# gcallipo/RadioDSP_SDR_RX

Hardware: AMD Instinct MI355X
Metric: IQ Msamples/s through full SSB+NR chain; achieved HBM GB/s vs peak (higher is better)
Workload: dtype f32

## Files before the change

radiodsp_sdr_rx_amd/csrc/rdsp_tail.hip:

```cpp
#include "rdsp_wave.h"

using namespace rdsp;

namespace {

typedef float v2f __attribute__((ext_vector_type(2)));

template <int CTRL>
__device__ __forceinline__ float dpp0_f(float v) {
  return __builtin_bit_cast(
      float, __builtin_amdgcn_update_dpp(0, __builtin_bit_cast(int, v), CTRL, 0xF, 0xF, true));
}

__device__ __forceinline__ float reduce_halves(float a0, float a1) {
  float t;
  asm("s_nop 1\n\t"
      "v_add_f32_dpp %0, %1, %1 row_ror:8 row_mask:0xf bank_mask:0x3\n\t"
      "v_add_f32_dpp %0, %2, %2 row_ror:8 row_mask:0xf bank_mask:0xc\n\t"
      "s_nop 1\n\t"
      "v_add_f32_dpp %0, %0, %0 row_half_mirror row_mask:0xf bank_mask:0xf\n\t"
      "s_nop 1\n\t"
      "v_add_f32_dpp %0, %0, %0 quad_perm:[2,3,0,1] row_mask:0xf bank_mask:0xf\n\t"
      "s_nop 1\n\t"
      "v_add_f32_dpp %0, %0, %0 quad_perm:[1,0,3,2] row_mask:0xf bank_mask:0xf"
      : "=&v"(t)
      : "v"(a0), "v"(a1));
  return t;
}

struct NlmsB {
  static constexpr int TPL = 6, GS = 64, SCR = 3 * GS;
  static constexpr int LDS_SCR = 2 * SCR;
  static constexpr bool OUT_IN_SCR = false;
  v2f w2[TPL / 2];
  v2f P[8];
  float energy;
  float emin;

  static __device__ __forceinline__ v2f pair_ld(const float *mine, int m) { return v2f{mine[m], mine[m + 1]}; }
  static __device__ __forceinline__ v2f pair_ld_even(const float *mine, int m) {
    typedef const volatile __attribute__((address_space(3))) v2f *LP;
    return *(LP)(mine + m);
  }
  __device__ __forceinline__ void load(const float *wst, const float *est, size_t ch, int sub) {
#pragma unroll
    for (int t = 0; t < TPL; t++) w2[t >> 1][t & 1] = wst[ch * RDSP_LMS_TAPS + (95 - (TPL * sub + t))];
    energy = est[ch];
    emin = __builtin_inff();
  }
  __device__ __forceinline__ void store(float *wst, float *est, size_t ch, int sub) {
#pragma unroll
    for (int t = 0; t < TPL; t++) wst[ch * RDSP_LMS_TAPS + (95 - (TPL * sub + t))] = w2[t >> 1][t & 1];
    if (sub == 0) est[ch] = energy;
  }

  static __device__ __forceinline__ void prepare(const float *cur, int s0, int sub, float mu, float e_base,
                                                 float b_base, float *dst, float &emin) {
    const float *x = cur + s0 + 4 * sub;
    const float xm = x[-1], qm = x[-97];
    const float4 xv = *reinterpret_cast<const float4 *>(x), qv = *reinterpret_cast<const float4 *>(x - 96);
    const float xs[5] = {xm, xv.x, xv.y, xv.z, xv.w}, qs[5] = {qm, qv.x, qv.y, qv.z, qv.w};
    float ea[4], ba[4];
#pragma unroll
    for (int k = 0; k < 4; k++) {
      const float de = fmaf(xs[k + 1], xs[k + 1], -(qs[k + 1] * qs[k + 1]));
      const float db = fmaf(xs[k + 1], xs[k], -(qs[k + 1] * qs[k]));
      ea[k] = (k == 0) ? de : ea[k - 1] + de;
      ba[k] = (k == 0) ? db : ba[k - 1] + db;
    }
    float ie = ea[3], ib = ba[3];
    ie += dpp0_f<0x111>(ie); ib += dpp0_f<0x111>(ib);
    ie += dpp0_f<0x112>(ie); ib += dpp0_f<0x112>(ib);
    ie += dpp0_f<0x114>(ie); ib += dpp0_f<0x114>(ib);
    ie += dpp0_f<0x118>(ie); ib += dpp0_f<0x118>(ib);
    const float oe = e_base + (ie - ea[3]), ob = b_base + (ib - ba[3]);
    float e[4], g[4], b[4];
#pragma unroll
    for (int k = 0; k < 4; k++) {
      e[k] = oe + ea[k];
      b[k] = ob + ba[k];
      const float den = e[k] + 0.000000119209289f;
      g[k] = mu * __builtin_amdgcn_rcpf(den);
      emin = fminf(emin, den);
    }
    float4 *d4 = reinterpret_cast<float4 *>(dst);
    d4[sub] = make_float4(g[0], g[1], g[2], g[3]);
    d4[GS / 4 + sub] = make_float4(b[0], b[1], b[2], b[3]);
    d4[GS / 2 + sub] = make_float4(e[0], e[1], e[2], e[3]);
  }

  template <bool OUT_E>
  __device__ __forceinline__ void block(const float *ring, bool first, float mu, float *out, float *scr, int sub, bool running) {
    const float *cur = ring + RDSP_BLOCK;
    const float *dsrc = first ? cur : ring;
    const float *mine = cur - TPL * sub;
    float bb = 0.f, ee = 0.f;
#pragma unroll
    for (int t = 0; t < TPL; t++) {
      bb = fmaf(mine[-1 - t], mine[-2 - t], bb);
      ee = fmaf(mine[-1 - t], mine[-1 - t], ee);
    }
    float b_base = row_allsum(bb);
    float e_base = row_allsum(ee);
    e_base = running ? energy : e_base;
    prepare(cur, 0, sub, mu, e_base, b_base, scr, emin);
#pragma unroll
    for (int m = -5; m <= 0; m++) P[m & 7] = (m & 1) ? pair_ld(mine, m) : pair_ld_even(mine, m);
#pragma unroll 1
    for (int s0 = 0; s0 < RDSP_BLOCK; s0 += GS) {
      const float *sc = scr + ((s0 / GS) & 1) * SCR;
      wg_sync<1>();
      float4 gq = *reinterpret_cast<const float4 *>(sc);
      float4 bq = *reinterpret_cast<const float4 *>(sc + GS);
      float4 dq = *reinterpret_cast<const float4 *>(dsrc + s0);
      e_base = sc[2 * GS + GS - 1];
      b_base = sc[GS + GS - 1];
      if (s0 + GS < RDSP_BLOCK) prepare(cur, s0 + GS, sub, mu, e_base, b_base, scr + (((s0 / GS) + 1) & 1) * SCR, emin);
#pragma unroll
      for (int q = 0; q < GS / 4; q++) {
        const float gi[4] = {gq.x, gq.y, gq.z, gq.w}, bn[4] = {bq.x, bq.y, bq.z, bq.w};
        const float dd[4] = {dq.x, dq.y, dq.z, dq.w};
        if (q < GS / 4 - 1) {
          gq = *reinterpret_cast<const float4 *>(sc + 4 * (q + 1));
          bq = *reinterpret_cast<const float4 *>(sc + GS + 4 * (q + 1));
          dq = *reinterpret_cast<const float4 *>(dsrc + s0 + 4 * (q + 1));
        }
        float o4[4];
#pragma unroll
        for (int h = 0; h < 2; h++) {
          const int n = 4 * q + 2 * h;
          if ((n + 3 < GS) || (s0 + GS < RDSP_BLOCK)) {
            P[(n + 1) & 7] = pair_ld(mine, s0 + n + 1);
            P[(n + 2) & 7] = pair_ld_even(mine, s0 + n + 2);
          }
          v2f acc = v2f{w2[0][0], w2[0][0]} * P[n & 7];
          acc = __builtin_elementwise_fma(v2f{w2[0][1], w2[0][1]}, P[(n - 1) & 7], acc);
          acc = __builtin_elementwise_fma(v2f{w2[1][0], w2[1][0]}, P[(n - 2) & 7], acc);
          acc = __builtin_elementwise_fma(v2f{w2[1][1], w2[1][1]}, P[(n - 3) & 7], acc);
          acc = __builtin_elementwise_fma(v2f{w2[2][0], w2[2][0]}, P[(n - 4) & 7], acc);
          acc = __builtin_elementwise_fma(v2f{w2[2][1], w2[2][1]}, P[(n - 5) & 7], acc);
          const float t = reduce_halves(acc[0], acc[1]);
          const float dA0 = dd[2 * h] - dpp_f<0x150>(t);
          const float dA1 = dd[2 * h + 1] - dpp_f<0x158>(t);
          const float g0 = dA0 * gi[2 * h];
          const float e1 = fmaf(-g0, bn[2 * h + 1], dA1);
          const float g1 = e1 * gi[2 * h + 1];
          o4[2 * h] = OUT_E ? dA0 : dd[2 * h] - dA0;
          o4[2 * h + 1] = OUT_E ? e1 : dd[2 * h + 1] - e1;
          const v2f gg0 = {g0, g0}, gg1 = {g1, g1};
#pragma unroll
          for (int kk = 0; kk < TPL / 2; kk++) {
            const v2f p0 = P[(n - 2 * kk - 1) & 7], p1 = P[(n - 2 * kk) & 7];
            w2[kk] = __builtin_elementwise_fma(gg0, __builtin_shufflevector(p0, p0, 1, 0), w2[kk]);
            w2[kk] = __builtin_elementwise_fma(gg1, __builtin_shufflevector(p1, p1, 1, 0), w2[kk]);
          }
        }
        *reinterpret_cast<float4 *>(out + s0 + 4 * q) = make_float4(o4[0], o4[1], o4[2], o4[3]);
        __builtin_amdgcn_sched_barrier(0);
      }
    }
    energy = e_base;
  }
  static __device__ __forceinline__ float4 out4(const float *out, const float *, int i) {
    return *reinterpret_cast<const float4 *>(out + i);
  }
};

#ifdef RDSP_EXPERIMENTAL
#include "rdsp_tail_lookahead.h"
#endif

template <typename NL>
__device__ __forceinline__ uint32_t nlms_health(const NL &f) {
  float z = f.energy * 0.f;
#pragma unroll
  for (int k = 0; k < NL::TPL / 2; k++) z = fmaf(f.w2[k][0], 0.f, fmaf(f.w2[k][1], 0.f, z));
  const float bad_e = row_allsum(f.emin <= 0.f ? 1.f : 0.f);
  const float nf = row_allsum(z);
  return (bad_e > 0.f ? 1u : 0u) | (nf == 0.f ? 0u : 2u);
}

#ifdef RDSP_TAIL_PROFILE
#define RDSP_TP(i) do { const long long tp_now = __builtin_readcyclecounter(); tp_acc[i] += tp_now - tp_last; tp_last = tp_now; } while (0)
#else
#define RDSP_TP(i) do { } while (0)
#endif

template <bool DUAL, typename NL>
__device__ __forceinline__ void tail_body(const RdspTailParams &p) {
#ifdef RDSP_TAIL_PROFILE
  long long tp_acc[4] = {0, 0, 0, 0}, tp_last = __builtin_readcyclecounter();
#endif
  constexpr int CPW = 4, SPL = RDSP_BLOCK / 16;
  constexpr int RINGS = DUAL ? 2 : 1;
  constexpr int FIN = NL::OUT_IN_SCR ? 0 : RDSP_BLOCK;
  constexpr int PER_CH0 = 2 * RINGS * RDSP_BLOCK + FIN + NL::LDS_SCR;
  constexpr int PER_CH = PER_CH0 + (96 - PER_CH0 % 64) % 64;
  static_assert(PER_CH % 64 == 32 && PER_CH % 4 == 0, "channel pitch in LDS");
  static_assert(!(DUAL && NL::OUT_IN_SCR), "the two-instance kernel hands a block on through `out`");
  __shared__ __attribute__((aligned(16))) float lds[CPW][PER_CH];
  if (p.prio == 1) __builtin_amdgcn_s_setprio(1);
  else if (p.prio == 2) __builtin_amdgcn_s_setprio(2);
  else if (p.prio == 3) __builtin_amdgcn_s_setprio(3);
  const int lane = threadIdx.x;
  const int cw = lane >> 4, sub = lane & 15;
  size_t ch = (size_t)p.ch_base + (size_t)blockIdx.x * CPW + cw;
  const bool valid = ch < (size_t)p.n_channels;
  if (!valid) ch = p.n_channels - 1;

  float *ringA = &lds[cw][0];
  float *ringB = DUAL ? &lds[cw][2 * RDSP_BLOCK] : ringA;
  float *fin = &lds[cw][2 * RINGS * RDSP_BLOCK];
  float *scr = &lds[cw][2 * RINGS * RDSP_BLOCK + FIN];

  const bool has_inst = DUAL || p.nr_on || p.als_mode;
  const bool one_is_nr = !DUAL && p.nr_on;
  float *o_w = one_is_nr ? p.nr_w : p.als_w;
  float *o_prev = one_is_nr ? p.nr_prev : p.als_prev;
  float *o_energy = one_is_nr ? p.nr_energy : p.als_energy;
  const float o_mu = one_is_nr ? p.nr_mu : p.als_mu;
  const int o_first = one_is_nr ? p.nr_first : p.als_first;
  const int o_mode = one_is_nr ? p.nr_mode : p.als_mode;

  NL nr, als;
  if constexpr (DUAL) {
    nr.load(p.nr_w, p.nr_energy, ch, sub);
    als.load(p.als_w, p.als_energy, ch, sub);
  } else if (has_inst) {
    als.load(o_w, o_energy, ch, sub);
  }
  float agc_g = p.st_scal[ch * 4 + 1];

  if constexpr (DUAL) {
#pragma unroll
    for (int k = 0; k < SPL; k++) {
      ringA[sub * SPL + k] = p.nr_prev[ch * RDSP_BLOCK + sub * SPL + k];
      ringB[sub * SPL + k] = p.als_prev[ch * RDSP_BLOCK + sub * SPL + k];
    }
  } else if (has_inst) {
#pragma unroll
    for (int k = 0; k < SPL; k++) ringA[sub * SPL + k] = o_prev[ch * RDSP_BLOCK + sub * SPL + k];
  }
  const float4 *src4 = reinterpret_cast<const float4 *>(p.mid + ch * p.mid_stride + sub * SPL);
  static_assert(SPL == 8, "two float4 per lane and block");
  float4 nx0 = src4[0], nx1 = src4[1];
  __builtin_amdgcn_s_waitcnt(0x0F70);
  if (p.n_blocks > 0) {
    float4 *dst4 = reinterpret_cast<float4 *>(ringA + RDSP_BLOCK + sub * SPL);
    dst4[0] = nx0;
    dst4[1] = nx1;
    if (p.n_blocks > 1) {
      nx0 = src4[RDSP_BLOCK / 4];
      nx1 = src4[RDSP_BLOCK / 4 + 1];
    }
  }

#pragma unroll 1
  for (int b = 0; b < p.n_blocks; b++) {
    wg_sync<1>();
    RDSP_TP(0);
    if constexpr (DUAL) {
      float *o = ringB + RDSP_BLOCK;
      nr.template block<false>(ringA, p.nr_first && b == 0, p.nr_mu, o, scr, sub, p.energy_running != 0);
      wg_sync<1>();
      if (p.nr_mode == 0) {
#pragma unroll
        for (int k = 0; k < SPL; k++) o[sub * SPL + k] = mul_1p1(o[sub * SPL + k]);
        wg_sync<1>();
      }
      if (p.als_mode == 1) als.template block<true>(ringB, p.als_first && b == 0, p.als_mu, fin, scr, sub, p.energy_running != 0);
      else als.template block<false>(ringB, p.als_first && b == 0, p.als_mu, fin, scr, sub, p.energy_running != 0);
    } else if (has_inst) {
      if (o_mode == 1) als.template block<true>(ringA, o_first && b == 0, o_mu, fin, scr, sub, p.energy_running != 0);
      else als.template block<false>(ringA, o_first && b == 0, o_mu, fin, scr, sub, p.energy_running != 0);
    }
    wg_sync<1>();
    RDSP_TP(1);
    float L[SPL];
#pragma unroll
    for (int k = 0; k < SPL / 4; k++) {
      const float4 a = has_inst ? NL::out4(fin, scr, sub * SPL + 4 * k)
                                : *reinterpret_cast<const float4 *>(ringA + RDSP_BLOCK + sub * SPL + 4 * k);
      L[4 * k] = a.x; L[4 * k + 1] = a.y; L[4 * k + 2] = a.z; L[4 * k + 3] = a.w;
    }
    if (!DUAL && has_inst && o_mode == 0) {
#pragma unroll
      for (int k = 0; k < SPL; k++) L[k] = mul_1p1(L[k]);
    }
    if (b + 1 < p.n_blocks) {
      float4 *r4 = reinterpret_cast<float4 *>(ringA + sub * SPL);
#pragma unroll
      for (int k = 0; k < SPL / 4; k++) r4[k] = r4[RDSP_BLOCK / 4 + k];
      if constexpr (DUAL) {
        float4 *q4 = reinterpret_cast<float4 *>(ringB + sub * SPL);
#pragma unroll
        for (int k = 0; k < SPL / 4; k++) q4[k] = q4[RDSP_BLOCK / 4 + k];
      }
      r4[RDSP_BLOCK / 4] = nx0;
      r4[RDSP_BLOCK / 4 + 1] = nx1;
      if (b + 2 < p.n_blocks) {
        const float4 *n4 = src4 + (size_t)(b + 2) * (RDSP_BLOCK / 4);
        nx0 = n4[0];
        nx1 = n4[1];
      }
    }
    RDSP_TP(2);
    if (p.raw_out) {
      if (valid) {
#pragma unroll
        for (int k = 0; k < SPL; k++)
          p.raw_out[ch * p.mid_stride + (size_t)b * RDSP_BLOCK + sub * SPL + k] = L[k];
      }
      wg_sync<1>();
      continue;
    }
    if (p.agc_on) {
      float pw = 0.f;
#pragma unroll
      for (int k = 0; k < SPL; k++) pw += L[k] * L[k] + L[k] * L[k];
      pw = row_allsum(pw);
      float pp = pw / (float)(2 * RDSP_BLOCK);
      float rms = __builtin_amdgcn_sqrtf(pp);
      float gt = fminf(0.25f * __builtin_amdgcn_rcpf(rms + 1e-6f), 100.0f);
      float coef = (gt < agc_g) ? p.agc_attack : p.agc_decay;
      float gn = agc_g + coef * (gt - agc_g);
#pragma unroll
      for (int k = 0; k < SPL; k++) {
        int i = sub * SPL + k;
        float gg = agc_g + (gn - agc_g) * ((float)(i + 1) / (float)RDSP_BLOCK);
        L[k] *= gg;
      }
      agc_g = gn;
    }
    if (valid) {
      size_t o = ch * p.out_stride + (size_t)b * RDSP_BLOCK + sub * SPL;
#pragma unroll
      for (int k = 0; k < SPL; k += 4) {
        uint4 wv;
        float l0 = L[k] * p.out_gain, l1 = L[k + 1] * p.out_gain, l2 = L[k + 2] * p.out_gain,
              l3 = L[k + 3] * p.out_gain;
        wv.x = pack_lr(l0, l0); wv.y = pack_lr(l1, l1); wv.z = pack_lr(l2, l2); wv.w = pack_lr(l3, l3);
        *reinterpret_cast<uint4 *>(p.out_i16 + o + k) = wv;
        if (p.out_f32) {
          p.out_f32[o + k] = make_float2(l0, l0);
          p.out_f32[o + k + 1] = make_float2(l1, l1);
          p.out_f32[o + k + 2] = make_float2(l2, l2);
          p.out_f32[o + k + 3] = make_float2(l3, l3);
        }
      }
    }
    wg_sync<1>();
    RDSP_TP(3);
  }
#ifdef RDSP_TAIL_PROFILE
  if (p.out_f32 == nullptr && blockIdx.x == 0 && threadIdx.x == 0)
    printf("tail phases (cycles per 128-step block): top %lld  nlms %lld  rotate %lld  agc/pack %lld\n", tp_acc[0] / p.n_blocks,
           tp_acc[1] / p.n_blocks, tp_acc[2] / p.n_blocks, tp_acc[3] / p.n_blocks);
#endif

  if (p.st_status && has_inst) {
    uint32_t h_nr = 0, h_als = 0;
    if constexpr (DUAL) {
      h_nr = nlms_health(nr);
      h_als = nlms_health(als);
    } else if (one_is_nr) {
      h_nr = nlms_health(als);
    } else {
      h_als = nlms_health(als);
    }
    if (valid && sub == 0) {
      if (h_nr) p.st_status[ch] |= h_nr;
      if (h_als) p.st_status[p.st_status_stride + ch] |= h_als;
    }
  }
  if (valid) {
    if constexpr (DUAL) {
      nr.store(p.nr_w, p.nr_energy, ch, sub);
      als.store(p.als_w, p.als_energy, ch, sub);
#pragma unroll
      for (int k = 0; k < SPL; k++) {
        p.nr_prev[ch * RDSP_BLOCK + sub * SPL + k] = ringA[RDSP_BLOCK + sub * SPL + k];
        p.als_prev[ch * RDSP_BLOCK + sub * SPL + k] = ringB[RDSP_BLOCK + sub * SPL + k];
      }
    } else if (has_inst) {
      als.store(o_w, o_energy, ch, sub);
#pragma unroll
      for (int k = 0; k < SPL; k++) o_prev[ch * RDSP_BLOCK + sub * SPL + k] = ringA[RDSP_BLOCK + sub * SPL + k];
    }
    if (sub == 0 && !p.raw_out) p.st_scal[ch * 4 + 1] = agc_g;
  }
}

__global__ void __launch_bounds__(64) rdsp_tail_dual_kernel(RdspTailParams p) { tail_body<true, NlmsB>(p); }

__global__ void __launch_bounds__(64) rdsp_tail_kernel(RdspTailParams p) {
  tail_body<false, NlmsB>(p);
}
#ifdef RDSP_EXPERIMENTAL
__global__ void __launch_bounds__(64) __attribute__((amdgpu_num_vgpr(64))) rdsp_tail_lookahead_kernel(RdspTailParams p) {
  tail_body<false, NlmsL>(p);
}
__global__ void __launch_bounds__(64) __attribute__((amdgpu_num_vgpr(64))) rdsp_tail_four_kernel(RdspTailParams p) {
  tail_body<false, NlmsQ>(p);
}
#endif

}

#ifdef RDSP_EXPERIMENTAL
extern "C" int rdsp_launch_tail_shift(const RdspTailParams *p, hipStream_t stream);
extern "C" int rdsp_launch_tail_layouts(const RdspTailParams *p, int variant, hipStream_t stream);
#endif

extern "C" int rdsp_launch_tail(const RdspTailParams *p, int variant, hipStream_t stream) {
  const int grid = (p->n_channels - p->ch_base + 3) / 4;
  const bool dual = p->nr_on && p->als_mode;
  if (variant == 100) {
    if (dual) hipLaunchKernelGGL(rdsp_tail_dual_kernel, dim3(grid), dim3(64), 0, stream, *p);
    else hipLaunchKernelGGL(rdsp_tail_kernel, dim3(grid), dim3(64), 0, stream, *p);
    return (int)hipGetLastError();
  }
#ifdef RDSP_EXPERIMENTAL
  if (variant == 104 || variant == 105) {
    if (dual) hipLaunchKernelGGL(rdsp_tail_dual_kernel, dim3(grid), dim3(64), 0, stream, *p);
    else if (variant == 104) hipLaunchKernelGGL(rdsp_tail_lookahead_kernel, dim3(grid), dim3(64), 0, stream, *p);
    else hipLaunchKernelGGL(rdsp_tail_four_kernel, dim3(grid), dim3(64), 0, stream, *p);
    return (int)hipGetLastError();
  }
  if (variant == 16) return rdsp_launch_tail_shift(p, stream);
  if (variant == 101 || variant == 102 || variant == 116 || variant == 108) return rdsp_launch_tail_layouts(p, variant, stream);
#endif
  return (int)hipErrorNotSupported;
}
```

Before: 237,000.

## Keep NLMS step scalars in registers via DPP broadcast and rotate LDS ring slots

Result: faster. 241,500 (median of 6 runs) (+1.9%).

```diff
diff --git a/radiodsp_sdr_rx_amd/csrc/rdsp_tail.hip b/radiodsp_sdr_rx_amd/csrc/rdsp_tail.hip
--- a/radiodsp_sdr_rx_amd/csrc/rdsp_tail.hip
+++ b/radiodsp_sdr_rx_amd/csrc/rdsp_tail.hip
@@ -1,3 +1,4 @@
+#include <utility>
 #include "rdsp_wave.h"
 
 using namespace rdsp;
@@ -10,6 +11,22 @@
 __device__ __forceinline__ float dpp0_f(float v) {
   return __builtin_bit_cast(
       float, __builtin_amdgcn_update_dpp(0, __builtin_bit_cast(int, v), CTRL, 0xF, 0xF, true));
+}
+
+template <int Q>
+__device__ __forceinline__ float mul_row_lane(float x, float g) {
+  static_assert(Q >= 0 && Q < 16, "a lane of the row");
+  return x * dpp_f<0x150 + Q>(g);
+}
+template <int Q>
+__device__ __forceinline__ float fnma_row_lane(float x, float b, float acc) {
+  static_assert(Q >= 0 && Q < 16, "a lane of the row");
+  asm("v_fmac_f32_dpp %0, %1, -%2 row_newbcast:%3 row_mask:0xf bank_mask:0xf" : "+v"(acc) : "v"(b), "v"(x), "n"(Q));
+  return acc;
+}
+template <typename F, int... Q>
+__device__ __forceinline__ void unrolled(F &&f, std::integer_sequence<int, Q...>) {
+  (f(std::integral_constant<int, Q>{}), ...);
 }
 
 __device__ __forceinline__ float reduce_halves(float a0, float a1) {
@@ -29,8 +46,8 @@
 }
 
 struct NlmsB {
-  static constexpr int TPL = 6, GS = 64, SCR = 3 * GS;
-  static constexpr int LDS_SCR = 2 * SCR;
+  static constexpr int TPL = 6, GS = 64;
+  static constexpr int LDS_SCR = 0;
   static constexpr bool OUT_IN_SCR = false;
   v2f w2[TPL / 2];
   v2f P[8];
@@ -54,8 +71,11 @@
     if (sub == 0) est[ch] = energy;
   }
 
-  static __device__ __forceinline__ void prepare(const float *cur, int s0, int sub, float mu, float e_base,
-                                                 float b_base, float *dst, float &emin) {
+  struct Scal {
+    float g[4], b[4], e3;
+  };
+  static __device__ __forceinline__ Scal prepare(const float *cur, int s0, int sub, float mu, float e_base,
+                                                 float b_base, float &emin) {
     const float *x = cur + s0 + 4 * sub;
     const float xm = x[-1], qm = x[-97];
     const float4 xv = *reinterpret_cast<const float4 *>(x), qv = *reinterpret_cast<const float4 *>(x - 96);
@@ -74,23 +94,21 @@
     ie += dpp0_f<0x114>(ie); ib += dpp0_f<0x114>(ib);
     ie += dpp0_f<0x118>(ie); ib += dpp0_f<0x118>(ib);
     const float oe = e_base + (ie - ea[3]), ob = b_base + (ib - ba[3]);
-    float e[4], g[4], b[4];
+    Scal r;
 #pragma unroll
     for (int k = 0; k < 4; k++) {
-      e[k] = oe + ea[k];
-      b[k] = ob + ba[k];
-      const float den = e[k] + 0.000000119209289f;
-      g[k] = mu * __builtin_amdgcn_rcpf(den);
+      const float e = oe + ea[k];
+      r.b[k] = ob + ba[k];
+      const float den = e + 0.000000119209289f;
+      r.g[k] = mu * __builtin_amdgcn_rcpf(den);
       emin = fminf(emin, den);
-    }
-    float4 *d4 = reinterpret_cast<float4 *>(dst);
-    d4[sub] = make_float4(g[0], g[1], g[2], g[3]);
-    d4[GS / 4 + sub] = make_float4(b[0], b[1], b[2], b[3]);
-    d4[GS / 2 + sub] = make_float4(e[0], e[1], e[2], e[3]);
+      r.e3 = e;
+    }
+    return r;
   }
 
   template <bool OUT_E>
-  __device__ __forceinline__ void block(const float *ring, bool first, float mu, float *out, float *scr, int sub, bool running) {
+  __device__ __forceinline__ void block(const float *ring, bool first, float mu, float *out, float *, int sub, bool running) {
     const float *cur = ring + RDSP_BLOCK;
     const float *dsrc = first ? cur : ring;
     const float *mine = cur - TPL * sub;
@@ -103,28 +121,19 @@
     float b_base = row_allsum(bb);
     float e_base = row_allsum(ee);
     e_base = running ? energy : e_base;
-    prepare(cur, 0, sub, mu, e_base, b_base, scr, emin);
+    Scal sc = prepare(cur, 0, sub, mu, e_base, b_base, emin), nx = sc;
 #pragma unroll
     for (int m = -5; m <= 0; m++) P[m & 7] = (m & 1) ? pair_ld(mine, m) : pair_ld_even(mine, m);
 #pragma unroll 1
     for (int s0 = 0; s0 < RDSP_BLOCK; s0 += GS) {
-      const float *sc = scr + ((s0 / GS) & 1) * SCR;
-      wg_sync<1>();
-      float4 gq = *reinterpret_cast<const float4 *>(sc);
-      float4 bq = *reinterpret_cast<const float4 *>(sc + GS);
       float4 dq = *reinterpret_cast<const float4 *>(dsrc + s0);
-      e_base = sc[2 * GS + GS - 1];
-      b_base = sc[GS + GS - 1];
-      if (s0 + GS < RDSP_BLOCK) prepare(cur, s0 + GS, sub, mu, e_base, b_base, scr + (((s0 / GS) + 1) & 1) * SCR, emin);
-#pragma unroll
-      for (int q = 0; q < GS / 4; q++) {
-        const float gi[4] = {gq.x, gq.y, gq.z, gq.w}, bn[4] = {bq.x, bq.y, bq.z, bq.w};
+      e_base = dpp_f<0x15F>(sc.e3);
+      b_base = dpp_f<0x15F>(sc.b[3]);
+      if (s0 + GS < RDSP_BLOCK) nx = prepare(cur, s0 + GS, sub, mu, e_base, b_base, emin);
+      unrolled([&](auto qc) __attribute__((always_inline)) {
+        constexpr int q = decltype(qc)::value;
         const float dd[4] = {dq.x, dq.y, dq.z, dq.w};
-        if (q < GS / 4 - 1) {
-          gq = *reinterpret_cast<const float4 *>(sc + 4 * (q + 1));
-          bq = *reinterpret_cast<const float4 *>(sc + GS + 4 * (q + 1));
-          dq = *reinterpret_cast<const float4 *>(dsrc + s0 + 4 * (q + 1));
-        }
+        if (q < GS / 4 - 1) dq = *reinterpret_cast<const float4 *>(dsrc + s0 + 4 * (q + 1));
         float o4[4];
 #pragma unroll
         for (int h = 0; h < 2; h++) {
@@ -142,9 +151,9 @@
           const float t = reduce_halves(acc[0], acc[1]);
           const float dA0 = dd[2 * h] - dpp_f<0x150>(t);
           const float dA1 = dd[2 * h + 1] - dpp_f<0x158>(t);
-          const float g0 = dA0 * gi[2 * h];
-          const float e1 = fmaf(-g0, bn[2 * h + 1], dA1);
-          const float g1 = e1 * gi[2 * h + 1];
+          const float g0 = mul_row_lane<q>(dA0, sc.g[2 * h]);
+          const float e1 = fnma_row_lane<q>(g0, sc.b[2 * h + 1], dA1);
+          const float g1 = mul_row_lane<q>(e1, sc.g[2 * h + 1]);
           o4[2 * h] = OUT_E ? dA0 : dd[2 * h] - dA0;
           o4[2 * h + 1] = OUT_E ? e1 : dd[2 * h + 1] - e1;
           const v2f gg0 = {g0, g0}, gg1 = {g1, g1};
@@ -157,7 +166,8 @@
         }
         *reinterpret_cast<float4 *>(out + s0 + 4 * q) = make_float4(o4[0], o4[1], o4[2], o4[3]);
         __builtin_amdgcn_sched_barrier(0);
-      }
+      }, std::make_integer_sequence<int, GS / 4>{});
+      sc = nx;
     }
     energy = e_base;
   }
@@ -194,7 +204,8 @@
   constexpr int CPW = 4, SPL = RDSP_BLOCK / 16;
   constexpr int RINGS = DUAL ? 2 : 1;
   constexpr int FIN = NL::OUT_IN_SCR ? 0 : RDSP_BLOCK;
-  constexpr int PER_CH0 = 2 * RINGS * RDSP_BLOCK + FIN + NL::LDS_SCR;
+  constexpr int SLOTS = 4;
+  constexpr int PER_CH0 = SLOTS * RINGS * RDSP_BLOCK + FIN + NL::LDS_SCR;
   constexpr int PER_CH = PER_CH0 + (96 - PER_CH0 % 64) % 64;
   static_assert(PER_CH % 64 == 32 && PER_CH % 4 == 0, "channel pitch in LDS");
   static_assert(!(DUAL && NL::OUT_IN_SCR), "the two-instance kernel hands a block on through `out`");
@@ -209,9 +220,9 @@
   if (!valid) ch = p.n_channels - 1;
 
   float *ringA = &lds[cw][0];
-  float *ringB = DUAL ? &lds[cw][2 * RDSP_BLOCK] : ringA;
-  float *fin = &lds[cw][2 * RINGS * RDSP_BLOCK];
-  float *scr = &lds[cw][2 * RINGS * RDSP_BLOCK + FIN];
+  float *ringB = DUAL ? &lds[cw][SLOTS * RDSP_BLOCK] : ringA;
+  float *fin = &lds[cw][SLOTS * RINGS * RDSP_BLOCK];
+  float *scr = &lds[cw][SLOTS * RINGS * RDSP_BLOCK + FIN];
 
   const bool has_inst = DUAL || p.nr_on || p.als_mode;
   const bool one_is_nr = !DUAL && p.nr_on;
@@ -255,24 +266,33 @@
     }
   }
 
+  int slot = 0;
 #pragma unroll 1
   for (int b = 0; b < p.n_blocks; b++) {
+    const float *rA = ringA + slot * RDSP_BLOCK;
     wg_sync<1>();
     RDSP_TP(0);
     if constexpr (DUAL) {
-      float *o = ringB + RDSP_BLOCK;
-      nr.template block<false>(ringA, p.nr_first && b == 0, p.nr_mu, o, scr, sub, p.energy_running != 0);
+      float *rB = ringB + slot * RDSP_BLOCK;
+      float *o = rB + RDSP_BLOCK;
+      nr.template block<false>(rA, p.nr_first && b == 0, p.nr_mu, o, scr, sub, p.energy_running != 0);
       wg_sync<1>();
       if (p.nr_mode == 0) {
 #pragma unroll
         for (int k = 0; k < SPL; k++) o[sub * SPL + k] = mul_1p1(o[sub * SPL + k]);
         wg_sync<1>();
       }
-      if (p.als_mode == 1) als.template block<true>(ringB, p.als_first && b == 0, p.als_mu, fin, scr, sub, p.energy_running != 0);
-      else als.template block<false>(ringB, p.als_first && b == 0, p.als_mu, fin, scr, sub, p.energy_running != 0);
+      if (slot == 2) {
+        const float4 *o4 = reinterpret_cast<const float4 *>(o + sub * SPL);
+        float4 *m4 = reinterpret_cast<float4 *>(ringB + sub * SPL);
+#pragma unroll
+        for (int k = 0; k < SPL / 4; k++) m4[k] = o4[k];
+      }
+      if (p.als_mode == 1) als.template block<true>(rB, p.als_first && b == 0, p.als_mu, fin, scr, sub, p.energy_running != 0);
+      else als.template block<false>(rB, p.als_first && b == 0, p.als_mu, fin, scr, sub, p.energy_running != 0);
     } else if (has_inst) {
-      if (o_mode == 1) als.template block<true>(ringA, o_first && b == 0, o_mu, fin, scr, sub, p.energy_running != 0);
-      else als.template block<false>(ringA, o_first && b == 0, o_mu, fin, scr, sub, p.energy_running != 0);
+      if (o_mode == 1) als.template block<true>(rA, o_first && b == 0, o_mu, fin, scr, sub, p.energy_running != 0);
+      else als.template block<false>(rA, o_first && b == 0, o_mu, fin, scr, sub, p.energy_running != 0);
     }
     wg_sync<1>();
     RDSP_TP(1);
@@ -280,24 +300,23 @@
 #pragma unroll
     for (int k = 0; k < SPL / 4; k++) {
       const float4 a = has_inst ? NL::out4(fin, scr, sub * SPL + 4 * k)
-                                : *reinterpret_cast<const float4 *>(ringA + RDSP_BLOCK + sub * SPL + 4 * k);
+                                : *reinterpret_cast<const float4 *>(rA + RDSP_BLOCK + sub * SPL + 4 * k);
       L[4 * k] = a.x; L[4 * k + 1] = a.y; L[4 * k + 2] = a.z; L[4 * k + 3] = a.w;
     }
     if (!DUAL && has_inst && o_mode == 0) {
 #pragma unroll
       for (int k = 0; k < SPL; k++) L[k] = mul_1p1(L[k]);
     }
+    slot = slot == 2 ? 0 : slot + 1;
     if (b + 1 < p.n_blocks) {
-      float4 *r4 = reinterpret_cast<float4 *>(ringA + sub * SPL);
-#pragma unroll
-      for (int k = 0; k < SPL / 4; k++) r4[k] = r4[RDSP_BLOCK / 4 + k];
-      if constexpr (DUAL) {
-        float4 *q4 = reinterpret_cast<float4 *>(ringB + sub * SPL);
-#pragma unroll
-        for (int k = 0; k < SPL / 4; k++) q4[k] = q4[RDSP_BLOCK / 4 + k];
-      }
-      r4[RDSP_BLOCK / 4] = nx0;
-      r4[RDSP_BLOCK / 4 + 1] = nx1;
+      float4 *r4 = reinterpret_cast<float4 *>(ringA + (slot + 1) * RDSP_BLOCK + sub * SPL);
+      r4[0] = nx0;
+      r4[1] = nx1;
+      if (slot == 2) {
+        float4 *m4 = reinterpret_cast<float4 *>(ringA + sub * SPL);
+        m4[0] = nx0;
+        m4[1] = nx1;
+      }
       if (b + 2 < p.n_blocks) {
         const float4 *n4 = src4 + (size_t)(b + 2) * (RDSP_BLOCK / 4);
         nx0 = n4[0];
@@ -374,18 +393,19 @@
     }
   }
   if (valid) {
+    const int last = p.n_blocks > 0 ? ((p.n_blocks - 1) % 3 + 1) * RDSP_BLOCK : 0;
     if constexpr (DUAL) {
       nr.store(p.nr_w, p.nr_energy, ch, sub);
       als.store(p.als_w, p.als_energy, ch, sub);
 #pragma unroll
       for (int k = 0; k < SPL; k++) {
-        p.nr_prev[ch * RDSP_BLOCK + sub * SPL + k] = ringA[RDSP_BLOCK + sub * SPL + k];
-        p.als_prev[ch * RDSP_BLOCK + sub * SPL + k] = ringB[RDSP_BLOCK + sub * SPL + k];
+        p.nr_prev[ch * RDSP_BLOCK + sub * SPL + k] = ringA[last + sub * SPL + k];
+        p.als_prev[ch * RDSP_BLOCK + sub * SPL + k] = ringB[last + sub * SPL + k];
       }
     } else if (has_inst) {
       als.store(o_w, o_energy, ch, sub);
 #pragma unroll
-      for (int k = 0; k < SPL; k++) o_prev[ch * RDSP_BLOCK + sub * SPL + k] = ringA[RDSP_BLOCK + sub * SPL + k];
+      for (int k = 0; k < SPL; k++) o_prev[ch * RDSP_BLOCK + sub * SPL + k] = ringA[last + sub * SPL + k];
     }
     if (sub == 0 && !p.raw_out) p.st_scal[ch * 4 + 1] = agc_g;
   }
```
